# David-Wobrock/image-processing-graph-laplacian

Hardware: AMD Instinct MI355X
Metric: filtered Mpixels/sec @ 4K img, 0.5% samples; PSNR vs PETSc ref (higher is better)
Workload: dtype f32 (f32 storage and accumulation; MFMA operands split into f16 hi+lo pairs = 22 significant bits)

## Files before the change

image-processing-graph-laplacian_amd/csrc/band_plan.hpp:

```cpp
#pragma once
#include <cstdint>
#include <vector>

#if defined(__HIP__) || defined(__CUDACC__)
#define GLF_BAND_HD __host__ __device__
#else
#define GLF_BAND_HD
#endif

namespace glf {

#ifndef BAND_MAXROWS_X
#define BAND_MAXROWS_X 128
#endif
constexpr int BAND_MAXROWS = BAND_MAXROWS_X;
constexpr int BAND_RMAX = 1023;
constexpr unsigned BAND_EMPTY = 0x0000FFFFu;
#ifndef BAND_PB_X
#define BAND_PB_X 2
#endif
#ifndef BAND_NW_X
#define BAND_NW_X 8
#endif
constexpr int BAND_PB = BAND_PB_X, BAND_NW = BAND_NW_X;
constexpr int BAND_HALF_SHIFT = 3, BAND_BLOCK_SHIFT = 4, BAND_PAIR = 2;

GLF_BAND_HD inline bool band_win_live(unsigned u) { return (u & 0xFFFFu) <= (u >> 16); }
GLF_BAND_HD inline bool band_win_has(unsigned u, int c) { return c >= (int)(u & 0xFFFFu) && c <= (int)(u >> 16); }
GLF_BAND_HD inline unsigned band_win_hull(unsigned u, unsigned v)
{
    if (!band_win_live(u)) return v;
    if (!band_win_live(v)) return u;
    const unsigned lo = (u & 0xFFFFu) < (v & 0xFFFFu) ? (u & 0xFFFFu) : (v & 0xFFFFu);
    const unsigned hi = (u >> 16) > (v >> 16) ? (u >> 16) : (v >> 16);
    return lo | (hi << 16);
}
GLF_BAND_HD inline void band_rows_hull(const unsigned *rowband, int r0, int n, int *alo, int *ahi)
{
    int lo = 0xFFFF, hi = -1;
    for (int w = 0; w < n; ++w) {
        const unsigned rb = rowband[r0 + w];
        if (!band_win_live(rb)) continue;
        lo = (int)(rb & 0xFFFFu) < lo ? (int)(rb & 0xFFFFu) : lo;
        hi = (int)(rb >> 16) > hi ? (int)(rb >> 16) : hi;
    }
    *alo = lo;
    *ahi = hi;
}
GLF_BAND_HD inline void band_cols_range(const int *gcol, int nc, int cmin, int cmax, int *lo, int *count)
{
    int l = 0, h = nc;
    while (l < h) {
        const int mid = (l + h) >> 1;
        if (gcol[mid] < cmin) l = mid + 1;
        else h = mid;
    }
    const int first = l;
    h = nc;
    while (l < h) {
        const int mid = (l + h) >> 1;
        if (gcol[mid] <= cmax) l = mid + 1;
        else h = mid;
    }
    *lo = first;
    *count = l - first;
}

struct BandGeom {
    int rad = 0;
    double D2 = 0.0;
    std::vector<int> rows, cols, dcmax;
    bool init(const int *grows, int nr, const int *gcols, int nc, double s_loc);
    unsigned band_of(int r) const;
    unsigned window(int cmin, int cmax, int dr, int shift) const;
};

}
```

image-processing-graph-laplacian_amd/csrc/nystroem_band.inc:

```

#ifndef BAND_SETPRIO
#define BAND_SETPRIO 1
#endif
#ifndef BAND_PCOPY
#define BAND_PCOPY 16
#endif
#ifndef BAND_NBUF
#define BAND_NBUF 2
#endif
constexpr unsigned BAND_PSTRIDE = 4u * BAND_PCOPY;
#ifndef BAND_GROWS
#define BAND_GROWS 4
#endif
constexpr int BAND_G = BAND_GROWS;
__host__ __device__ constexpr inline int band_chunk_bytes(int mb) { return mb * 2048 + 256; }
constexpr int BAND_WB = 6;
__host__ __device__ constexpr inline int band_stage_chunks(bool samples)
{
    return samples && 2 * BAND_WB > BAND_NBUF * BAND_G ? 2 * BAND_WB : BAND_NBUF * BAND_G;
}
__host__ __device__ inline unsigned band_lds_bytes(int mb, int nw, int rad, int ksc, bool samples, bool plut = true)
{
    return (plut ? 256u * BAND_PSTRIDE : 0u) + (unsigned)band_stage_chunks(samples) * (unsigned)band_chunk_bytes(mb) + 4u * (unsigned)(rad + 1) + 64u * (unsigned)ksc + 4u * BAND_MAXROWS * (unsigned)(1 + 2 * nw) + 16u;
}
// ... 464 lines not shown
        if (qblk[BAND_NBUF - 1] <= Bhi) issued = issue(qblk[BAND_NBUF - 1], qg0[BAND_NBUF - 1], (buf + BAND_NBUF - 1) % BAND_NBUF);
        if (wvalid || noskip) {
            if (blk != cur_blk) {
                cur_blk = blk;
#pragma unroll
                for (int e = 0; e < 8; ++e) {
                    const int cb = SAMPLES ? gcs[16 * blk + 8 * half + e] : gcs[8 * blk + e];
#pragma unroll
                    for (int b = 0; b < PB; ++b) ec[b][e >> 1][e & 1] = elut[min(abs(tc[b] - cb), rad)];
                }
            }
#pragma unroll 1
            for (int slot = 0; slot < BAND_G; ++slot) {
                const int i = g0 + RP * slot;
                if (i >= nb) break;
                const unsigned u = (unsigned)__builtin_amdgcn_readfirstlane((int)wwin[wave * BAND_MAXROWS + i]);
                if (!noskip && !band_win_has(u, blk)) continue;
                ++nsteps;
                const unsigned char *sl = stage + (size_t)(buf * BAND_G + slot) * CHB;
                const int ie = SAMPLES ? i : i + half;
                const float era = ie < nb ? er_s[wave * BAND_MAXROWS + ie] : 0.f;
                kstep(sl, era, ec);
            }
        }
        if (BAND_NBUF > 2) dma_wait(issued);
        else lds_dma_drain();
        __syncthreads();
#pragma unroll
        for (int d = 0; d < BAND_NBUF - 1; ++d) {
            qblk[d] = qblk[d + 1];
            qg0[d] = qg0[d + 1];
        }
        if (qblk[BAND_NBUF - 1] <= Bhi) advance(qblk[BAND_NBUF - 1], qg0[BAND_NBUF - 1]);
        blk = qblk[0];
        g0 = qg0[0];
        buf = (buf + 1) % BAND_NBUF;
    }
    if (evaluated && lane == 0 && nsteps) atomicAdd(evaluated, nsteps * (unsigned long long)(16 * 32 * PB));

    float iv[MB], csum[MB];
#pragma unroll
    for (int j = 0; j < MB; ++j) {
        iv[j] = inv[32 * j + l31];
        csum[j] = 0.f;
    }
    if (GREY && !SAMPLES && fw) {
        if (wvalid) {
            BandFilter flt;
            flt.sig = fsig;
            flt.w = fw;
            flt.gain = fgain;
            flt.ysub = fysub;
            flt.out = fout;
            flt.zf = fzf;
            flt.corr = fcorr;
            float wv[1 + NS][MB];
#pragma unroll
            for (int k = 0; k <= NS; ++k)
#pragma unroll
                for (int j = 0; j < MB; ++j) wv[k][j] = (k == 0 ? flt.w[32 * j + l31] : flt.sig.w[(k - 1) * LD + 32 * j + l31]) * iv[j];
#pragma unroll
            for (int b = 0; b < PB; ++b) {
#pragma unroll
                for (int q = 0; q < 16; ++q) {
                    float sdot[1 + NS];
#pragma unroll
                    for (int k = 0; k <= NS; ++k) {
                        sdot[k] = 0.f;
#pragma unroll
                        for (int j = 0; j < MB; ++j) sdot[k] = fmaf(acc[b][j][q], wv[k][j], sdot[k]);
#pragma unroll
                        for (int o = 16; o > 0; o >>= 1) sdot[k] += __shfl_xor(sdot[k], o, 64);
                    }
                    const int col = (tile * PB + b) * 32 + (q & 3) + 8 * (q >> 2) + 4 * half;
                    if (l31 == 0 && col < width) {
                        const int64_t px = (int64_t)trow * width + col;
                        if (mask[px]) continue;
                        band_filter_store<1 + NS>(flt, fpix0, px, (int)tval[px], sdot);
                    }
                }
            }
        }
        return;
    }
    if (wvalid) {
#pragma unroll
        for (int b = 0; b < PB; ++b) {
#pragma unroll
            for (int q = 0; q < 16; ++q) {
                const int t = (q & 3) + 8 * (q >> 2) + 4 * half;
                if (SAMPLES) {
                    const int bi = tile * 32 + t;
                    if (bi >= nc) continue;
                    const size_t s = (size_t)trow * nc + bi;
                    const float dg = (float)degree[s];
#pragma unroll
                    for (int j = 0; j < MB; ++j)
                        out[s * out_ld + 32 * j + l31] = alpha * fmaf(dg, X[s * x_ld + 32 * j + l31], -(acc[b][j][q] * iv[j]));
                } else {
                    const int col = (tile * PB + b) * 32 + t;
                    if (col >= width) continue;
                    const int64_t px = (int64_t)trow * width + col;
                    const bool is_sample = mask[px] != 0;
                    int64_t dst;
                    if (raster) dst = px;
                    else {
                        if (is_sample) continue;
                        dst = (int64_t)p + px - (int64_t)samples_before(idx, p, (uint32_t)px);
                    }
                    const float yv = (!GREY || is_sample) ? 0.f : (float)tval[px];
#pragma unroll
                    for (int j = 0; j < MB; ++j) {
                        const float v = acc[b][j][q] * iv[j];
                        out[(size_t)dst * out_ld + 32 * j + l31] = v;
                        csum[j] = fmaf(v, yv, csum[j]);
                    }
                }
            }
        }
    }
    if (GREY && !SAMPLES && cpartial) {
        __syncthreads();
        float *red = reinterpret_cast<float *>(stage);
#pragma unroll
        for (int j = 0; j < MB; ++j) {
            const float v = csum[j] + __shfl_xor(csum[j], 32, 64);
            if (half == 0) red[wave * LD + 32 * j + l31] = v;
        }
        __syncthreads();
        if (tid < LD) {
            double tot = 0.0;
            for (int w = 0; w < NW; ++w) tot += (double)red[w * LD + tid];
            cpartial[((size_t)blockIdx.y * gridDim.x + blockIdx.x) * LD + tid] = tot;
        }
    }
}

struct BandTables {
    int rad = 0, nr = 0, nc = 0, ksc = 0, width = 0;
    int tile_px = 0, ntiles_px = 0, ntiles_s = 0;
    bool ok = false;
    DevBuf<unsigned> blob;
    size_t o_pexp = 0, o_grid = 0, o_rb_px = 0, o_win_px = 0, o_rb_s = 0, o_win_s = 0, o_dcmax = 0;
    const float *tab() const { return reinterpret_cast<const float *>(blob.p); }
    const float *pexp() const { return reinterpret_cast<const float *>(blob.p + o_pexp); }
    const int *grow() const { return reinterpret_cast<const int *>(blob.p + o_grid); }
    const int *gcol() const { return grow() + nr; }
    const unsigned *rowband_px() const { return blob.p + o_rb_px; }
    const unsigned *win_px() const { return blob.p + o_win_px; }
    const unsigned *rowband_s() const { return blob.p + o_rb_s; }
    const unsigned *win_s() const { return blob.p + o_win_s; }
    const int *dcmax() const { return reinterpret_cast<const int *>(blob.p + o_dcmax); }
    std::vector<unsigned> h_rowband_px;
    int dc0() const { return geom.dcmax.empty() ? -1 : geom.dcmax[0]; }
    int cols_near_tile(int t) const
    {
        int lo = 0, n = 0;
        if (dc0() >= 0) band_cols_range(geom.cols.data(), nc, t * tile_px - dc0(), std::min(width, (t + 1) * tile_px) - 1 + dc0(), &lo, &n);
        return n;
    }
    std::vector<double> pairs_dr;
    std::vector<double> pairs_dr_s;
    std::vector<int> hrows;
    BandGeom geom;
    unsigned band_of(int r) const { return geom.band_of(r); }
    double pairs_rows(const std::vector<double> &per_dr, int r) const
    {
        const unsigned rb = band_of(r);
        double tot = 0.0;
        for (int a = (int)(rb & 0xFFFFu); a <= (int)(rb >> 16); ++a) tot += per_dr[std::abs(r - hrows[a])];
        return tot;
    }
    mutable int memo_r0 = -1, memo_r1 = -1;
    mutable double memo_pairs = 0.0;
    double pairs_px(int row0, int row1) const
    {
        if (row0 == memo_r0 && row1 == memo_r1) return memo_pairs;
        double tot = 0.0;
        for (int r = row0; r < row1; ++r) tot += pairs_rows(pairs_dr, r);
        memo_r0 = row0;
        memo_r1 = row1;
        memo_pairs = tot;
        return tot;
    }
    double pairs_s(int a0, int a1) const
    {
        double tot = 0.0;
        for (int t = a0; t < a1; ++t) tot += pairs_rows(pairs_dr_s, hrows[t]);
        return tot;
    }
    int build(glf_ctx *ctx, const GridInfo &g, KernelCoef coef, int width_, int height, int tile_px_, bool want_px, bool want_s)
    {
        ok = false;
        if (!geom.init(g.rows.data(), g.nr, g.cols.data(), g.nc, (double)coef.s_loc)) return GLF_ERR_UNSUPPORTED;
        rad = geom.rad;
        nr = g.nr;
        nc = g.nc;
        ksc = (int)ceil_div(nc, 16);
        width = width_;
        tile_px = tile_px_;
        hrows = g.rows;
        if (nr > 65535 || ksc > 65535) return GLF_ERR_UNSUPPORTED;
        ntiles_px = want_px ? (int)ceil_div(width, tile_px) : 0;
        ntiles_s = want_s ? (int)ceil_div(nc, 32) : 0;
        const size_t n_tab = 256 + 2 * (size_t)(rad + 1);
        o_pexp = (n_tab + 3) / 4 * 4;
        o_grid = o_pexp + 256 * (size_t)BAND_PCOPY;
        o_rb_px = o_grid + (size_t)nr + nc;
        o_win_px = o_rb_px + (want_px ? (size_t)height : 0);
        o_rb_s = o_win_px + (size_t)rad * ntiles_px;
        o_win_s = o_rb_s + (want_s ? (size_t)nr : 0);
        o_dcmax = o_win_s + (size_t)rad * ntiles_s;
        std::vector<unsigned> h(o_dcmax + (size_t)rad);
        float *htab = reinterpret_cast<float *>(h.data());
        for (int e = 0; e < 256; ++e) htab[e] = (float)std::exp2(-(double)coef.s_val * e * e);
        for (int d = 0; d <= rad; ++d) {
            const double t = (double)coef.s_loc * (double)d * (double)d;
            htab[256 + d] = d < rad ? (float)std::exp2(-t) : 0.f;
            htab[256 + rad + 1 + d] = d < rad ? (float)std::exp2((double)NYS_F16_KSCALE_LOG2 - t) : 0.f;
        }
        for (int i = 0; i < 256 * BAND_PCOPY; ++i) reinterpret_cast<float *>(h.data())[o_pexp + i] = htab[i / BAND_PCOPY];
        for (int a = 0; a < nr; ++a) h[o_grid + a] = (unsigned)g.rows[a];
        for (int b = 0; b < nc; ++b) h[o_grid + nr + b] = (unsigned)g.cols[b];
        const std::vector<int> &dcmax = geom.dcmax;
        for (int dr = 0; dr < rad; ++dr) h[o_dcmax + dr] = (unsigned)dcmax[dr];
        int maxband = 0;
        if (want_px) {
            for (int r = 0; r < height; ++r) {
                const unsigned rb = band_of(r);
                h[o_rb_px + r] = rb;
                maxband = std::max(maxband, (int)(rb >> 16) - (int)(rb & 0xFFFF) + 1);
            }
            h_rowband_px.assign(h.begin() + o_rb_px, h.begin() + o_win_px);
            for (int dr = 0; dr < rad; ++dr)
                for (int t = 0; t < ntiles_px; ++t) h[o_win_px + (size_t)dr * ntiles_px + t] = geom.window(t * tile_px, std::min(width, (t + 1) * tile_px) - 1, dr, BAND_HALF_SHIFT);
            pairs_dr.assign(rad, 0.0);
            for (int dr = 0; dr < rad; ++dr) {
                if (dcmax[dr] < 0) continue;
                double n = 0.0;
                for (int b = 0; b < nc; ++b) n += (double)(std::min(width - 1, g.cols[b] + dcmax[dr]) - std::max(0, g.cols[b] - dcmax[dr]) + 1);
                pairs_dr[dr] = n;
            }
        }
        if (want_s) {
            for (int a = 0; a < nr; ++a) {
                const unsigned rb = band_of(g.rows[a]);
                h[o_rb_s + a] = rb;
                maxband = std::max(maxband, (int)(rb >> 16) - (int)(rb & 0xFFFF) + 1);
            }
            for (int dr = 0; dr < rad; ++dr)
                for (int t = 0; t < ntiles_s; ++t) h[o_win_s + (size_t)dr * ntiles_s + t] = geom.window(g.cols[t * 32], g.cols[std::min(nc, (t + 1) * 32) - 1], dr, BAND_BLOCK_SHIFT);
            pairs_dr_s.assign(rad, 0.0);
            for (int dr = 0; dr < rad; ++dr) {
                if (dcmax[dr] < 0) continue;
                double n = 0.0;
                int lo = 0, hi = 0;
                for (int b = 0; b < nc; ++b) {
                    while (lo < nc && g.cols[lo] < g.cols[b] - dcmax[dr]) ++lo;
                    while (hi < nc && g.cols[hi] <= g.cols[b] + dcmax[dr]) ++hi;
                    n += (double)(hi - lo);
                }
                pairs_dr_s[dr] = n;
            }
        }
        if (maxband + 8 > BAND_MAXROWS) return GLF_ERR_UNSUPPORTED;
        GLF_TRY(blob.alloc(ctx, h.size()));
        GLF_HIP(ctx, hipMemcpyAsync(blob.p, h.data(), sizeof(unsigned) * h.size(), hipMemcpyHostToDevice, ctx->stream));
        GLF_HIP(ctx, hipStreamSynchronize(ctx->stream));
        ok = true;
        return GLF_OK;
    }
    bool narrow(int height) const { return 2.0 * rad < 0.5 * std::min(width, height); }
};

struct BandCacheEntry {
    BandTables bt;
    std::vector<int> rows, cols;
    float s_loc = 0.f, s_val = 0.f;
    int width = 0, height = 0, tile_px = 0;
};
static void band_cache_delete(void *e) { delete reinterpret_cast<BandCacheEntry *>(e); }
static int band_tables_cached(glf_ctx *ctx, const GridInfo &g, KernelCoef coef, int width, int height, int tile_px, bool px, const BandTables **out)
{
    using Entry = BandCacheEntry;
    Entry *&e = reinterpret_cast<Entry *&>(ctx->band_cache[px ? 0 : 1]);
    if (e && e->bt.ok && e->rows == g.rows && e->cols == g.cols && e->s_loc == coef.s_loc && e->s_val == coef.s_val && e->width == width &&
        e->height == height && e->tile_px == tile_px) {
        *out = &e->bt;
        return GLF_OK;
    }
    delete e;
    e = new Entry;
    e->rows = g.rows;
    e->cols = g.cols;
    e->s_loc = coef.s_loc;
    e->s_val = coef.s_val;
    e->width = width;
    e->height = height;
    e->tile_px = tile_px;
    const int rc = e->bt.build(ctx, g, coef, width, height, tile_px, px, !px);
    if (rc != GLF_OK) {
        delete e;
        e = nullptr;
        return rc;
    }
    *out = &e->bt;
    return GLF_OK;
}

#ifndef BAND_NW_S_X
#define BAND_NW_S_X 8
#endif
constexpr int BAND_NW_S = BAND_NW_S_X;

template <int MB, int NS = 0, PixGen G = PixGen::Grey>
static int launch_band_px(glf_ctx *ctx, const BandTables &bt, const uint8_t *d_img, int row0, int nrows, const unsigned char *chunks,
                          const float *inv, float *phi, int phi_ld, const uint8_t *d_mask, const uint32_t *d_idx, unsigned p, int raster,
                          double *cpartial, unsigned long long *evaluated, const BandFilter *flt = nullptr, int64_t pix0 = 0, float nsval = 0.f)
{
    if constexpr (G != PixGen::Grey)
        if (flt || cpartial) return set_error(ctx, GLF_ERR_INVALID, "k_band: the colour and 16-bit formats have no filter epilogue");
    if constexpr (NS == 0 && G == PixGen::Grey)
        if (flt && flt->sig.nsig > 0) {
            if (flt->sig.nsig >= BANDV_MAXNC) return set_error(ctx, GLF_ERR_INVALID, "k_band: %d signal planes", flt->sig.nsig);
            return band_dispatch_planes(1 + flt->sig.nsig, [&](auto nc) -> int {
                return launch_band_px<MB, decltype(nc)::value - 1>(ctx, bt, d_img, row0, nrows, chunks, inv, phi, phi_ld, d_mask, d_idx, p, raster,
                                                                   cpartial, evaluated, flt, pix0);
            });
        }
    auto kern = k_band<MB, BAND_PB, BAND_NW, false, NS, G>;
    const unsigned lds = band_lds_bytes(MB, BAND_NW, bt.rad, bt.ksc, false, G == PixGen::Grey);
    GLF_HIP(ctx, hipFuncSetAttribute(reinterpret_cast<const void *>(kern), hipFuncAttributeMaxDynamicSharedMemorySize, (int)lds));
    const dim3 grid((unsigned)bt.ntiles_px, (unsigned)ceil_div(nrows, BAND_NW));
    hipLaunchKernelGGL(kern, grid, dim3(BAND_NW * 64), lds, ctx->stream, d_img, bt.width, row0, bt.grow(), bt.gcol(), bt.nr, bt.nc,
                       bt.ksc, bt.tab(), bt.pexp(), bt.rad, bt.rowband_px(), bt.win_px(), bt.ntiles_px, chunks, inv, phi, phi_ld, d_mask, d_idx, p, raster,
                       cpartial, (const float *)nullptr, 0, (const double *)nullptr, 0.f, evaluated, row0 + nrows, flt ? flt->w : (const float *)nullptr,
                       flt ? flt->gain : 0.f, flt ? flt->ysub : 0.f, flt ? flt->out : (uint8_t *)nullptr, flt ? flt->zf : (float *)nullptr,
                       flt ? flt->corr : (float *)nullptr, pix0, flt ? flt->sig : BandSignals{}, ctx->tune.band_noskip ? 1 : 0, nsval);
    GLF_LAUNCH_CHECK(ctx);
    return GLF_OK;
}
inline size_t band_px_wgs(const BandTables &bt, int nrows) { return (size_t)bt.ntiles_px * (size_t)ceil_div(nrows, BAND_NW); }

template <int MB, PixGen G = PixGen::Grey>
static int launch_band_samples(glf_ctx *ctx, const BandTables &bt, const uint8_t *svals, int a0, int nrows, const unsigned char *chunks,
                               const float *inv, float *Y, int y_ld, const float *X, int x_ld, const double *degree, float alpha,
                               unsigned long long *evaluated, float nsval = 0.f)
{
    auto kern = k_band<MB, 1, BAND_NW_S, true, 0, G>;
    const unsigned lds = band_lds_bytes(MB, BAND_NW_S, bt.rad, bt.ksc, true, G == PixGen::Grey);
    GLF_HIP(ctx, hipFuncSetAttribute(reinterpret_cast<const void *>(kern), hipFuncAttributeMaxDynamicSharedMemorySize, (int)lds));
    const dim3 grid((unsigned)bt.ntiles_s, (unsigned)ceil_div(nrows, BAND_NW_S));
    hipLaunchKernelGGL(kern, grid, dim3(BAND_NW_S * 64), lds, ctx->stream, svals, bt.nc, a0, bt.grow(), bt.gcol(), bt.nr, bt.nc, bt.ksc,
                       bt.tab(), bt.pexp(), bt.rad, bt.rowband_s(), bt.win_s(), bt.ntiles_s, chunks, inv, Y, y_ld, (const uint8_t *)nullptr,
                       (const uint32_t *)nullptr, 0u, 1, (double *)nullptr, X, x_ld, degree, alpha, evaluated, a0 + nrows, (const float *)nullptr, 0.f,
                       0.f, (uint8_t *)nullptr, (float *)nullptr, (float *)nullptr, (int64_t)0, BandSignals{}, 0, nsval);
    GLF_LAUNCH_CHECK(ctx);
    return GLF_OK;
}

static int band_prep(glf_ctx *ctx, const float *X, unsigned x_ld, const float *colscale, const void *svals, bool raw, int nr, int nc, int ksc, int mb,
                     unsigned char *chunks, int nch = 1)
{
    const size_t total = (size_t)nr * ksc * mb * 64;
    auto kern = raw && nch == 3 ? k_band_prep<true, 3> : raw ? k_band_prep<true> : k_band_prep<false>;
    hipLaunchKernelGGL(kern, dim3((unsigned)ceil_div((int64_t)total, 256)), dim3(256), 0, ctx->stream, X, x_ld, colscale, svals, nr, nc, ksc, mb, chunks);
    GLF_LAUNCH_CHECK(ctx);
    return GLF_OK;
}

static int band_svals(glf_ctx *ctx, const float4 *d_samples, unsigned p, DevBuf<uint8_t> &svals)
{
    GLF_TRY(svals.alloc(ctx, p));
    hipLaunchKernelGGL(k_gridop_svals, dim3((p + 255) / 256), dim3(256), 0, ctx->stream, d_samples, p, svals.p);
    GLF_LAUNCH_CHECK(ctx);
    return GLF_OK;
}
static int band_eval_zero(glf_ctx *ctx, DevBuf<unsigned long long> &dev_eval)
{
    GLF_TRY(dev_eval.alloc(ctx, 1));
    GLF_HIP(ctx, hipMemsetAsync(dev_eval.p, 0, sizeof(unsigned long long), ctx->stream));
    return GLF_OK;
}
static int band_eval_read(glf_ctx *ctx, const DevBuf<unsigned long long> &dev_eval, unsigned long long *h_eval)
{
    unsigned long long *pin_eval = ctx_pinned(ctx) ? reinterpret_cast<unsigned long long *>(ctx_pinned(ctx) + PINNED_BANDEVAL) : nullptr;
// ... 116 lines not shown
```

image-processing-graph-laplacian_amd/csrc/nystroem_band_sep.inc:

```

constexpr int BSEP_RB = 8;
constexpr int BSEP_ATILE = 128;
constexpr size_t BSEP_S_BYTES = 256u << 20;
static_assert(BSEP_RB == BAND_NW, "a block of the row pass is the rows of one workgroup of the column pass");
static_assert(BSEP_ATILE >= BAND_MAXROWS, "without BAND_NOSKIP one tile holds the band of a block of rows");

template <int NC>
__global__ __launch_bounds__(256) void k_band_sep_g(const float *__restrict__ psi, unsigned p, unsigned ld, const float *__restrict__ w,
                                                    const float *__restrict__ sig_w, const uint8_t *__restrict__ svals,
                                                    const float *__restrict__ ftab, int R, float *__restrict__ G)
{
    const unsigned s = blockIdx.x * 256 + threadIdx.x;
    if (s >= p) return;
    double acc[NC];
    band_q_row<NC>(psi + (size_t)s * ld, ld, w, sig_w, acc);
    const int v = (int)svals[s];
    for (int t = 0; t < R; t += 4) {
        const float f0 = ftab[(t + 0) * 256 + v], f1 = ftab[(t + 1) * 256 + v], f2 = ftab[(t + 2) * 256 + v], f3 = ftab[(t + 3) * 256 + v];
#pragma unroll
        for (int k = 0; k < NC; ++k) {
            const float q = (float)acc[k];
            *reinterpret_cast<float4 *>(G + ((size_t)k * p + s) * R + t) = make_float4(f0 * q, f1 * q, f2 * q, f3 * q);
        }
    }
}

__global__ __launch_bounds__(256) void k_band_sep_rows(const float *__restrict__ G, unsigned E, unsigned ncR, int nr, int row_begin, int row_end,
                                                       int srow0, const int *__restrict__ grow, const float *__restrict__ btab, int rad,
                                                       const unsigned *__restrict__ rowband, int noskip, float *__restrict__ S)
{
    __shared__ __attribute__((aligned(16))) float er_l[BSEP_ATILE][BSEP_RB];
    const int r0 = row_begin + blockIdx.y * BSEP_RB, nrb = min(BSEP_RB, row_end - r0);
    int alo, ahi;
    band_rows_hull(rowband, r0, nrb, &alo, &ahi);
    if (noskip) {
        alo = 0;
        ahi = nr - 1;
    }
    const unsigned e = blockIdx.x * 256 + threadIdx.x;
    const bool live = e < E;
    const unsigned plane = live ? e / ncR : 0u, rem = live ? e - plane * ncR : 0u;
    const float *g = G + (size_t)plane * nr * ncR + rem;
    float acc[BSEP_RB];
#pragma unroll
    for (int j = 0; j < BSEP_RB; ++j) acc[j] = 0.f;
    for (int a0 = alo; a0 <= ahi; a0 += BSEP_ATILE) {
        const int na = min(BSEP_ATILE, ahi - a0 + 1);
        __syncthreads();
        for (int i = threadIdx.x; i < na * BSEP_RB; i += 256) {
            const int dr = min(abs(r0 + i % BSEP_RB - grow[a0 + i / BSEP_RB]), rad);
            er_l[i / BSEP_RB][i % BSEP_RB] = btab[256 + rad + 1 + dr];
        }
        __syncthreads();
        if (live)
            for (int i = 0; i < na; ++i) {
                const float gv = g[(size_t)(a0 + i) * ncR];
                const float4 e0 = *reinterpret_cast<const float4 *>(&er_l[i][0]), e1 = *reinterpret_cast<const float4 *>(&er_l[i][4]);
                const float er[BSEP_RB] = {e0.x, e0.y, e0.z, e0.w, e1.x, e1.y, e1.z, e1.w};
#pragma unroll
                for (int j = 0; j < BSEP_RB; ++j) acc[j] = fmaf(er[j], gv, acc[j]);
            }
    }
    if (live)
#pragma unroll
        for (int j = 0; j < BSEP_RB; ++j)
            if (j < nrb) S[(size_t)(r0 + j - srow0) * E + e] = acc[j];
}

__host__ __device__ inline unsigned band_sep_lds_bytes(int R, int rad) { return 4u * (256u * (unsigned)(R + 1) + (unsigned)(rad + 1)); }

template <int NC, int KB>
__global__ __launch_bounds__(BAND_NW * 64) void k_band_sep_cols(const uint8_t *__restrict__ img, int width, int row_begin, int row_end, int srow0,
                                                                const int *__restrict__ gcol, int nc, const float *__restrict__ btab, int rad,
                                                                int dc0, const float *__restrict__ S, int R, const float *__restrict__ ftab,
                                                                const uint8_t *__restrict__ mask, BandFilter flt, int64_t fpix0, int noskip)
{
    constexpr int NW = BAND_NW;
    extern __shared__ __attribute__((aligned(16))) unsigned char bsdyn[];
    float *ft = reinterpret_cast<float *>(bsdyn);
    float *elut = ft + 256 * (R + 1);
    const int tid = threadIdx.x, lane = tid & 63, wave = __builtin_amdgcn_readfirstlane(tid >> 6);
    const int trow0 = row_begin + blockIdx.y * NW, ntw = min(NW, row_end - trow0);
    const int tc0 = blockIdx.x * 64, tc1 = min(width, tc0 + 64) - 1;
    for (int i = tid; i < 256 * R; i += NW * 64) ft[(i & 255) * (R + 1) + (i >> 8)] = ftab[i];
    for (int i = tid; i <= rad; i += NW * 64) elut[i] = btab[256 + i];
    int Clo = 0, W = 0;
    if (dc0 >= 0) band_cols_range(gcol, nc, tc0 - dc0, tc1 + dc0, &Clo, &W);
    __syncthreads();
    if (wave >= ntw && !noskip) return;
    const int trow = min(trow0 + wave, row_end - 1), tcol = min(tc0 + lane, width - 1);
    const int pv = (int)img[(size_t)trow * width + tcol];
    const float *fpx = ft + pv * (R + 1);
    const size_t ncR = (size_t)nc * R;
    double tot[NC];
#pragma unroll
    for (int k = 0; k < NC; ++k) {
        tot[k] = 0.0;
        const float *Srow = S + ((size_t)(trow - srow0) * NC + k) * ncR + (size_t)Clo * R;
        for (int k0 = 0; k0 < R; k0 += KB) {
            float U[KB];
#pragma unroll
            for (int t = 0; t < KB; ++t) U[t] = 0.f;
            for (int bb = 0; bb < W; ++bb) {
                const float ecv = elut[min(abs(tcol - gcol[Clo + bb]), rad)];
                const float *sp = Srow + (size_t)bb * R + k0;
#pragma unroll
                for (int t = 0; t < KB; ++t) U[t] = fmaf(ecv, sp[t], U[t]);
            }
#pragma unroll
            for (int t = 0; t < KB; ++t) tot[k] = fma((double)fpx[k0 + t], (double)U[t], tot[k]);
        }
    }

    if (wave >= ntw || tc0 + lane >= width) return;
    const int64_t px = (int64_t)trow * width + tcol;
    if (mask[px]) return;
    float sdot[NC];
#pragma unroll
    for (int k = 0; k < NC; ++k) sdot[k] = (float)(tot[k] * BAND_UNSCALE);
    band_filter_store<NC>(flt, fpix0, px, pv, sdot);
}

template <int NC, int KB>
static int band_sep_cols_launch(glf_ctx *ctx, const BandTables &bt, const uint8_t *d_img, int row0, int nrows, int srow0, const float *S, int R,
                                const float *ftab, unsigned lds, const uint8_t *d_mask, const BandFilter &flt, int64_t pix0)
{
    auto kern = k_band_sep_cols<NC, KB>;
    if (lds > 48u * 1024u) GLF_HIP(ctx, hipFuncSetAttribute(reinterpret_cast<const void *>(kern), hipFuncAttributeMaxDynamicSharedMemorySize, (int)lds));
    const dim3 grid((unsigned)bt.ntiles_px, (unsigned)ceil_div(nrows, BAND_NW));
    hipLaunchKernelGGL(kern, grid, dim3(BAND_NW * 64), lds, ctx->stream, d_img, bt.width, row0, row0 + nrows, srow0, bt.gcol(), bt.nc, bt.tab(), bt.rad,
                       bt.dc0(), S, R, ftab, d_mask, flt, pix0, ctx->tune.band_noskip ? 1 : 0);
    GLF_LAUNCH_CHECK(ctx);
    return GLF_OK;
}

static int launch_nystroem_band_sep(glf_ctx *ctx, const BandTables &bt, const uint8_t *d_img, int width, int64_t pix0, int64_t pix1,
                                    const float4 *d_samples, const uint8_t *d_mask, unsigned p, KernelCoef coef, const float *d_psi, unsigned ld,
                                    const BandFilter &flt, float *kernel_ms, uint64_t *entries_evaluated, double *mfma_flops, RowpassStats *stats)
{
    const int row0 = (int)(pix0 / width), row1 = (int)(pix1 / width), nrows = row1 - row0;
    const int ncol = 1 + flt.sig.nsig;
    if (ncol < 1 || ncol > BANDV_MAXNC || bt.width != width || p != (unsigned)bt.nr * (unsigned)bt.nc) return GLF_ERR_UNSUPPORTED;
    int R = 0;
    const float *ftab = nullptr;
    const _Float16 *Ff = nullptr;
    GLF_TRY(rank_tables(ctx, coef, &R, &ftab, &Ff));
    if (R <= 0) return GLF_ERR_UNSUPPORTED;
    const unsigned lds = band_sep_lds_bytes(R, bt.rad);
    if (lds > BANDV_LDS_MAX) return GLF_ERR_UNSUPPORTED;
    const size_t row_bytes = sizeof(float) * (size_t)bt.nc * R * ncol;
    int chunk = (int)std::min<size_t>((size_t)round_up(nrows, BAND_NW), std::max<size_t>(BAND_NW, BSEP_S_BYTES / row_bytes / BAND_NW * BAND_NW));
    DevBuf<uint8_t> svals;
    DevBuf<float> G, S;
    GLF_TRY(G.alloc(ctx, (size_t)ncol * p * R));
    while (S.alloc(ctx, (size_t)chunk * bt.nc * R * ncol) != GLF_OK) {
        if (chunk <= BAND_NW) return GLF_ERR_NOMEM;
        chunk = (int)round_up(chunk / 2, BAND_NW);
    }
    GLF_TRY(band_svals(ctx, d_samples, p, svals));
    hipStream_t st = ctx->stream;
    hipEvent_t e0 = ctx->ev[6], e1 = ctx->ev[7];
    const bool noskip = ctx->tune.band_noskip;
    GLF_TRY(band_dispatch_planes(ncol, [&](auto nc_) -> int {
        constexpr int NC = decltype(nc_)::value;
        hipLaunchKernelGGL(k_band_sep_g<NC>, dim3((p + 255) / 256), dim3(256), 0, st, d_psi, p, ld, flt.w, flt.sig.w, svals.p, ftab, R, G.p);
        GLF_LAUNCH_CHECK(ctx);
        const unsigned ncR = (unsigned)bt.nc * (unsigned)R, E = ncR * NC;
        GLF_HIP(ctx, hipEventRecord(e0, st));
        for (int c0 = 0; c0 < nrows; c0 += chunk) {
            const int r0 = row0 + c0, n = std::min(chunk, nrows - c0);
            hipLaunchKernelGGL(k_band_sep_rows, dim3((E + 255) / 256, (unsigned)ceil_div(n, BSEP_RB)), dim3(256), 0, st, G.p, E, ncR, bt.nr, r0, r0 + n, r0,
                               bt.grow(), bt.tab(), bt.rad, bt.rowband_px(), noskip ? 1 : 0, S.p);
            GLF_LAUNCH_CHECK(ctx);
            if (R % 32 == 0) GLF_TRY((band_sep_cols_launch<NC, 32>(ctx, bt, d_img, r0, n, r0, S.p, R, ftab, lds, d_mask, flt, pix0)));
            else GLF_TRY((band_sep_cols_launch<NC, 16>(ctx, bt, d_img, r0, n, r0, S.p, R, ftab, lds, d_mask, flt, pix0)));
        }
        GLF_HIP(ctx, hipEventRecord(e1, st));
        return GLF_OK;
    }));
    GLF_HIP(ctx, hipStreamSynchronize(st));
    float ms = 0.f;
    GLF_HIP(ctx, hipEventElapsedTime(&ms, e0, e1));
    if (kernel_ms) *kernel_ms = ms;
    if (entries_evaluated) {
        uint64_t cols = 0, rows = 0;
        for (int t = 0; t < bt.ntiles_px; ++t) cols += (uint64_t)bt.cols_near_tile(t);
        if (noskip) rows = (uint64_t)ceil_div(nrows, BAND_NW) * BAND_NW * (uint64_t)bt.nr;
        else
            for (int r = row0; r < row1; ++r) {
                int alo, ahi;
                band_rows_hull(bt.h_rowband_px.data(), r, 1, &alo, &ahi);
                rows += (uint64_t)std::max(0, ahi - alo + 1);
            }
        *entries_evaluated = 64ull * cols * rows;
    }
    if (mfma_flops) *mfma_flops = 0.0;
    band_stats(stats, bt, row0, row1, 1, ms, (unsigned)ncol, R);
    return GLF_OK;
}
```

Baseline: 2512.

## Move separable band column pass onto split-f16 MFMA with per-plane scaling

```diff
diff --git a/image-processing-graph-laplacian_amd/csrc/band_plan.hpp b/image-processing-graph-laplacian_amd/csrc/band_plan.hpp
--- a/image-processing-graph-laplacian_amd/csrc/band_plan.hpp
+++ b/image-processing-graph-laplacian_amd/csrc/band_plan.hpp
@@ -66,6 +66,33 @@
     *count = l - first;
 }
 
+constexpr int BSEP_KSTEP = 16;
+GLF_BAND_HD inline void band_sep_tile_cols(const int *gcol, int nc, int width, int tc0, int tile_px, int d, int *clo, int *count)
+{
+    *clo = 0;
+    *count = 0;
+    const int tc1 = (tc0 + tile_px < width ? tc0 + tile_px : width) - 1;
+    if (d >= 0 && tc1 >= tc0) band_cols_range(gcol, nc, tc0 - d, tc1 + d, clo, count);
+}
+GLF_BAND_HD inline int band_sep_ksteps(int count) { return (count + BSEP_KSTEP - 1) / BSEP_KSTEP; }
+GLF_BAND_HD inline int band_sep_col(int clo, int i, int nc) { return clo + i < nc - 1 ? clo + i : nc - 1; }
+GLF_BAND_HD inline bool band_sep_block_dead(const int *gcol, int nc, int clo, int count, int ks, int p0, int p1, int rad)
+{
+    const int i1 = BSEP_KSTEP * ks + BSEP_KSTEP - 1 < count - 1 ? BSEP_KSTEP * ks + BSEP_KSTEP - 1 : count - 1;
+    const int first = gcol[band_sep_col(clo, BSEP_KSTEP * ks, nc)], last = gcol[band_sep_col(clo, i1, nc)];
+    return first - p1 >= rad || p0 - last >= rad;
+}
+GLF_BAND_HD inline uint64_t band_sep_tile_entries(const int *gcol, int nc, int width, int tc0, int tile_px, int d, int rad, bool all)
+{
+    int clo, count;
+    band_sep_tile_cols(gcol, nc, width, tc0, tile_px, d, &clo, &count);
+    uint64_t n = 0;
+    for (int ks = 0; ks < band_sep_ksteps(count); ++ks)
+        for (int pt = 0; pt < tile_px / 32; ++pt)
+            if (all || !band_sep_block_dead(gcol, nc, clo, count, ks, tc0 + 32 * pt, tc0 + 32 * pt + 31, rad)) n += (uint64_t)BSEP_KSTEP * 32u;
+    return n;
+}
+
 struct BandGeom {
     int rad = 0;
     double D2 = 0.0;
diff --git a/image-processing-graph-laplacian_amd/csrc/nystroem_band.inc b/image-processing-graph-laplacian_amd/csrc/nystroem_band.inc
--- a/image-processing-graph-laplacian_amd/csrc/nystroem_band.inc
+++ b/image-processing-graph-laplacian_amd/csrc/nystroem_band.inc
@@ -640,6 +640,7 @@
     const unsigned *win_s() const { return blob.p + o_win_s; }
     const int *dcmax() const { return reinterpret_cast<const int *>(blob.p + o_dcmax); }
     std::vector<unsigned> h_rowband_px;
+    double er15_rowsum = 0.0;
     int dc0() const { return geom.dcmax.empty() ? -1 : geom.dcmax[0]; }
     int cols_near_tile(int t) const
     {
@@ -720,6 +721,13 @@
                 maxband = std::max(maxband, (int)(rb >> 16) - (int)(rb & 0xFFFF) + 1);
             }
             h_rowband_px.assign(h.begin() + o_rb_px, h.begin() + o_win_px);
+            er15_rowsum = 0.0;
+            for (int r = 0; r < height; ++r) {
+                const unsigned rb = h[o_rb_px + r];
+                double s = 0.0;
+                for (int a = (int)(rb & 0xFFFFu); a <= (int)(rb >> 16); ++a) s += (double)htab[256 + rad + 1 + std::min(std::abs(r - g.rows[a]), rad)];
+                er15_rowsum = std::max(er15_rowsum, s);
+            }
             for (int dr = 0; dr < rad; ++dr)
                 for (int t = 0; t < ntiles_px; ++t) h[o_win_px + (size_t)dr * ntiles_px + t] = geom.window(t * tile_px, std::min(width, (t + 1) * tile_px) - 1, dr, BAND_HALF_SHIFT);
             pairs_dr.assign(rad, 0.0);
diff --git a/image-processing-graph-laplacian_amd/csrc/nystroem_band_sep.inc b/image-processing-graph-laplacian_amd/csrc/nystroem_band_sep.inc
--- a/image-processing-graph-laplacian_amd/csrc/nystroem_band_sep.inc
+++ b/image-processing-graph-laplacian_amd/csrc/nystroem_band_sep.inc
@@ -8,12 +8,23 @@
 template <int NC>
 __global__ __launch_bounds__(256) void k_band_sep_g(const float *__restrict__ psi, unsigned p, unsigned ld, const float *__restrict__ w,
                                                     const float *__restrict__ sig_w, const uint8_t *__restrict__ svals,
-                                                    const float *__restrict__ ftab, int R, float *__restrict__ G)
-{
+                                                    const float *__restrict__ ftab, int R, float *__restrict__ G, float *__restrict__ qpart)
+{
+    __shared__ float qm[4][NC];
     const unsigned s = blockIdx.x * 256 + threadIdx.x;
-    if (s >= p) return;
+    const bool live = s < p;
     double acc[NC];
-    band_q_row<NC>(psi + (size_t)s * ld, ld, w, sig_w, acc);
+    if (live) band_q_row<NC>(psi + (size_t)s * ld, ld, w, sig_w, acc);
+#pragma unroll
+    for (int k = 0; k < NC; ++k) {
+        float m = live ? fabsf((float)acc[k]) : 0.f;
+#pragma unroll
+        for (int o = 32; o > 0; o >>= 1) m = fmaxf(m, __shfl_xor(m, o, 64));
+        if ((threadIdx.x & 63) == 0) qm[threadIdx.x >> 6][k] = m;
+    }
+    __syncthreads();
+    if (threadIdx.x < NC) qpart[(size_t)blockIdx.x * NC + threadIdx.x] = fmaxf(fmaxf(qm[0][threadIdx.x], qm[1][threadIdx.x]), fmaxf(qm[2][threadIdx.x], qm[3][threadIdx.x]));
+    if (!live) return;
     const int v = (int)svals[s];
     for (int t = 0; t < R; t += 4) {
         const float f0 = ftab[(t + 0) * 256 + v], f1 = ftab[(t + 1) * 256 + v], f2 = ftab[(t + 2) * 256 + v], f3 = ftab[(t + 3) * 256 + v];
@@ -67,69 +78,187 @@
             if (j < nrb) S[(size_t)(r0 + j - srow0) * E + e] = acc[j];
 }
 
+constexpr int BSEP_EC_LOG2 = 12;
+__global__ __launch_bounds__(256) void k_band_sep_scales(const float *__restrict__ qpart, int nblk, int ncol, float er15_rowsum, float *__restrict__ scl)
+{
+    __shared__ float sh[256];
+    for (int k = 0; k < ncol; ++k) {
+        float m = 0.f;
+        for (int i = threadIdx.x; i < nblk; i += 256) m = fmaxf(m, qpart[(size_t)i * ncol + k]);
+        __syncthreads();
+        sh[threadIdx.x] = m;
+        __syncthreads();
+        for (int o = 128; o > 0; o >>= 1) {
+            if ((int)threadIdx.x < o) sh[threadIdx.x] = fmaxf(sh[threadIdx.x], sh[threadIdx.x + o]);
+            __syncthreads();
+        }
+        if (threadIdx.x == 0) {
+            const float mx = sh[0] * er15_rowsum;
+            int e = 0;
+            if (mx > 0.f && isfinite(mx)) {
+                int ex;
+                (void)frexpf(mx, &ex);
+                e = 14 - ex;
+            }
+            e = max(-90, min(90, e));
+            scl[k] = ldexpf(1.0f, e);
+            scl[BANDV_MAXNC + k] = ldexpf(1.0f, -e - BSEP_EC_LOG2);
+        }
+    }
+}
+
+#ifndef BSEP_PT_X
+#define BSEP_PT_X 4
+#endif
+constexpr int BSEP_PT = BSEP_PT_X;
+constexpr int BSEP_KCH = 4;
+static_assert(BSEP_PT % 2 == 0 && BSEP_PT >= 2 && BSEP_PT <= 8, "a lane ends with BSEP_PT / 2 pixels");
+
 __host__ __device__ inline unsigned band_sep_lds_bytes(int R, int rad) { return 4u * (256u * (unsigned)(R + 1) + (unsigned)(rad + 1)); }
-
-template <int NC, int KB>
-__global__ __launch_bounds__(BAND_NW * 64) void k_band_sep_cols(const uint8_t *__restrict__ img, int width, int row_begin, int row_end, int srow0,
-                                                                const int *__restrict__ gcol, int nc, const float *__restrict__ btab, int rad,
-                                                                int dc0, const float *__restrict__ S, int R, const float *__restrict__ ftab,
-                                                                const uint8_t *__restrict__ mask, BandFilter flt, int64_t fpix0, int noskip)
-{
-    constexpr int NW = BAND_NW;
+__host__ __device__ inline unsigned band_sep_frag_offset(int R, int rad) { return (band_sep_lds_bytes(R, rad) + 15u) & ~15u; }
+__host__ __device__ inline unsigned band_sep_mfma_lds_bytes(int R, int rad) { return band_sep_frag_offset(R, rad) + (unsigned)(BSEP_KCH * BSEP_PT) * 2048u; }
+
+template <int NC, int PT>
+__global__ __launch_bounds__(BAND_NW * 64) void k_band_sep_cols_mfma(const uint8_t *__restrict__ img, int width, int row_begin, int row_end, int srow0,
+                                                                     const int *__restrict__ gcol, int nc, const float *__restrict__ btab, int rad,
+                                                                     int dc0, const float *__restrict__ S, int R, const float *__restrict__ ftab,
+                                                                     const float *__restrict__ scl, const uint8_t *__restrict__ mask, BandFilter flt,
+                                                                     int64_t fpix0, int noskip)
+{
+    constexpr int NW = BAND_NW, NI = PT / 2;
     extern __shared__ __attribute__((aligned(16))) unsigned char bsdyn[];
     float *ft = reinterpret_cast<float *>(bsdyn);
     float *elut = ft + 256 * (R + 1);
-    const int tid = threadIdx.x, lane = tid & 63, wave = __builtin_amdgcn_readfirstlane(tid >> 6);
+    f16x8 *bfrag = reinterpret_cast<f16x8 *>(bsdyn + band_sep_frag_offset(R, rad));
+    const int tid = threadIdx.x, lane = tid & 63, wave = __builtin_amdgcn_readfirstlane(tid >> 6), half = lane >> 5, l31 = lane & 31;
     const int trow0 = row_begin + blockIdx.y * NW, ntw = min(NW, row_end - trow0);
-    const int tc0 = blockIdx.x * 64, tc1 = min(width, tc0 + 64) - 1;
+    const int tc0 = blockIdx.x * (32 * PT);
     for (int i = tid; i < 256 * R; i += NW * 64) ft[(i & 255) * (R + 1) + (i >> 8)] = ftab[i];
     for (int i = tid; i <= rad; i += NW * 64) elut[i] = btab[256 + i];
-    int Clo = 0, W = 0;
-    if (dc0 >= 0) band_cols_range(gcol, nc, tc0 - dc0, tc1 + dc0, &Clo, &W);
+    int Clo, W;
+    band_sep_tile_cols(gcol, nc, width, tc0, 32 * PT, dc0, &Clo, &W);
+    const int nks = band_sep_ksteps(W);
+    const bool walk = wave < ntw || noskip;
+    const int trow = min(trow0 + wave, row_end - 1);
+    int pv[PT];
+#pragma unroll
+    for (int t = 0; t < PT; ++t) pv[t] = (int)img[(size_t)trow * width + min(tc0 + 32 * t + l31, width - 1)];
     __syncthreads();
-    if (wave >= ntw && !noskip) return;
-    const int trow = min(trow0 + wave, row_end - 1), tcol = min(tc0 + lane, width - 1);
-    const int pv = (int)img[(size_t)trow * width + tcol];
-    const float *fpx = ft + pv * (R + 1);
+    auto form = [&](int ks0) {
+        for (int i = tid; i < BSEP_KCH * PT * 64; i += NW * 64) {
+            const int ln = i & 63, t = (i >> 6) % PT, ks = ks0 + (i >> 6) / PT;
+            if (ks >= nks) break;
+            const int cpx = tc0 + 32 * t + (ln & 31);
+            f16x8 hi, lo;
+#pragma unroll
+            for (int j = 0; j < 8; ++j) {
+                const int e = BSEP_KSTEP * ks + 8 * (ln >> 5) + j;
+                const float ec = elut[min(abs(cpx - gcol[band_sep_col(Clo, e, nc)]), rad)];
+                const float v = e < W ? ec * (float)(1 << BSEP_EC_LOG2) : 0.f;
+                hi[j] = (_Float16)v;
+                lo[j] = (_Float16)(v - (float)hi[j]);
+            }
+            bfrag[((i >> 6) * 2 + 0) * 64 + ln] = hi;
+            bfrag[((i >> 6) * 2 + 1) * 64 + ln] = lo;
+        }
+    };
+    const bool once = nks <= BSEP_KCH;
+    if (once) {
+        form(0);
+        __syncthreads();
+    }
     const size_t ncR = (size_t)nc * R;
-    double tot[NC];
-#pragma unroll
+    float sdot[NI][NC];
+#pragma unroll 1
     for (int k = 0; k < NC; ++k) {
-        tot[k] = 0.0;
-        const float *Srow = S + ((size_t)(trow - srow0) * NC + k) * ncR + (size_t)Clo * R;
-        for (int k0 = 0; k0 < R; k0 += KB) {
-            float U[KB];
-#pragma unroll
-            for (int t = 0; t < KB; ++t) U[t] = 0.f;
-            for (int bb = 0; bb < W; ++bb) {
-                const float ecv = elut[min(abs(tcol - gcol[Clo + bb]), rad)];
-                const float *sp = Srow + (size_t)bb * R + k0;
-#pragma unroll
-                for (int t = 0; t < KB; ++t) U[t] = fmaf(ecv, sp[t], U[t]);
-            }
-#pragma unroll
-            for (int t = 0; t < KB; ++t) tot[k] = fma((double)fpx[k0 + t], (double)U[t], tot[k]);
-        }
-    }
-
-    if (wave >= ntw || tc0 + lane >= width) return;
-    const int64_t px = (int64_t)trow * width + tcol;
-    if (mask[px]) return;
-    float sdot[NC];
-#pragma unroll
-    for (int k = 0; k < NC; ++k) sdot[k] = (float)(tot[k] * BAND_UNSCALE);
-    band_filter_store<NC>(flt, fpix0, px, pv, sdot);
-}
-
-template <int NC, int KB>
+        const float sc = scl[k];
+        const float *Srow = S + ((size_t)(trow - srow0) * NC + k) * ncR;
+        double tot[PT];
+#pragma unroll
+        for (int t = 0; t < PT; ++t) tot[t] = 0.0;
+        for (int k0 = 0; k0 < R; k0 += 32) {
+            f32x16 acc[PT];
+#pragma unroll
+            for (int t = 0; t < PT; ++t)
+#pragma unroll
+                for (int q = 0; q < 16; ++q) acc[t][q] = 0.f;
+            const bool kin = k0 + l31 < R;
+            const float *Sk = Srow + min(k0 + l31, R - 1);
+            for (int ks0 = 0; ks0 < nks; ks0 += BSEP_KCH) {
+                if (!once) {
+                    __syncthreads();
+                    form(ks0);
+                    __syncthreads();
+                }
+                if (!walk) continue;
+                const int ks1 = min(ks0 + BSEP_KCH, nks);
+                float sv[8], sn[8];
+#pragma unroll
+                for (int j = 0; j < 8; ++j) sn[j] = Sk[(size_t)band_sep_col(Clo, BSEP_KSTEP * ks0 + 8 * half + j, nc) * R];
+                for (int ks = ks0; ks < ks1; ++ks) {
+#pragma unroll
+                    for (int j = 0; j < 8; ++j) sv[j] = sn[j];
+                    if (ks + 1 < ks1)
+#pragma unroll
+                        for (int j = 0; j < 8; ++j) sn[j] = Sk[(size_t)band_sep_col(Clo, BSEP_KSTEP * (ks + 1) + 8 * half + j, nc) * R];
+                    f16x8 ah, al;
+#pragma unroll
+                    for (int j = 0; j < 8; ++j) {
+                        const float v = kin ? sv[j] * sc : 0.f;
+                        ah[j] = (_Float16)v;
+                        al[j] = (_Float16)(v - (float)ah[j]);
+                    }
+                    const f16x8 *bf = bfrag + (size_t)(ks - ks0) * PT * 128 + lane;
+#pragma unroll
+                    for (int t = 0; t < PT; ++t) {
+                        if (!noskip && band_sep_block_dead(gcol, nc, Clo, W, ks, tc0 + 32 * t, tc0 + 32 * t + 31, rad)) continue;
+                        const f16x8 bh = bf[t * 128], bl = bf[t * 128 + 64];
+                        acc[t] = __builtin_amdgcn_mfma_f32_32x32x16_f16(ah, bh, acc[t], 0, 0, 0);
+                        acc[t] = __builtin_amdgcn_mfma_f32_32x32x16_f16(ah, bl, acc[t], 0, 0, 0);
+                        acc[t] = __builtin_amdgcn_mfma_f32_32x32x16_f16(al, bh, acc[t], 0, 0, 0);
+                    }
+                }
+            }
+#pragma unroll
+            for (int q = 0; q < 16; ++q) {
+                if (k0 + 8 * (q >> 2) >= R) continue;
+                const int kk = k0 + (q & 3) + 8 * (q >> 2) + 4 * half;
+#pragma unroll
+                for (int t = 0; t < PT; ++t) tot[t] = fma((double)ft[pv[t] * (R + 1) + kk], (double)acc[t][q], tot[t]);
+            }
+        }
+        const double unscale = BAND_UNSCALE * (double)scl[BANDV_MAXNC + k];
+#pragma unroll
+        for (int i = 0; i < NI; ++i) {
+            const double s0 = tot[2 * i] + __shfl_xor(tot[2 * i], 32, 64), s1 = tot[2 * i + 1] + __shfl_xor(tot[2 * i + 1], 32, 64);
+            const float r = (float)((half ? s1 : s0) * unscale);
+#pragma unroll
+            for (int kk = 0; kk < NC; ++kk)
+                if (kk == k) sdot[i][kk] = r;
+        }
+    }
+
+    if (wave >= ntw) return;
+#pragma unroll
+    for (int i = 0; i < NI; ++i) {
+        const int col = tc0 + 64 * i + lane;
+        if (col >= width) continue;
+        const int64_t px = (int64_t)trow * width + col;
+        if (mask[px]) continue;
+        band_filter_store<NC>(flt, fpix0, px, (int)img[px], sdot[i]);
+    }
+}
+
+template <int NC>
 static int band_sep_cols_launch(glf_ctx *ctx, const BandTables &bt, const uint8_t *d_img, int row0, int nrows, int srow0, const float *S, int R,
-                                const float *ftab, unsigned lds, const uint8_t *d_mask, const BandFilter &flt, int64_t pix0)
-{
-    auto kern = k_band_sep_cols<NC, KB>;
+                                const float *ftab, const float *scl, const uint8_t *d_mask, const BandFilter &flt, int64_t pix0)
+{
+    auto kern = k_band_sep_cols_mfma<NC, BSEP_PT>;
+    const unsigned lds = band_sep_mfma_lds_bytes(R, bt.rad);
     if (lds > 48u * 1024u) GLF_HIP(ctx, hipFuncSetAttribute(reinterpret_cast<const void *>(kern), hipFuncAttributeMaxDynamicSharedMemorySize, (int)lds));
-    const dim3 grid((unsigned)bt.ntiles_px, (unsigned)ceil_div(nrows, BAND_NW));
+    const dim3 grid((unsigned)ceil_div(bt.width, 32 * BSEP_PT), (unsigned)ceil_div(nrows, BAND_NW));
     hipLaunchKernelGGL(kern, grid, dim3(BAND_NW * 64), lds, ctx->stream, d_img, bt.width, row0, row0 + nrows, srow0, bt.gcol(), bt.nc, bt.tab(), bt.rad,
-                       bt.dc0(), S, R, ftab, d_mask, flt, pix0, ctx->tune.band_noskip ? 1 : 0);
+                       bt.dc0(), S, R, ftab, scl, d_mask, flt, pix0, ctx->tune.band_noskip ? 1 : 0);
     GLF_LAUNCH_CHECK(ctx);
     return GLF_OK;
 }
@@ -146,12 +275,14 @@
     const _Float16 *Ff = nullptr;
     GLF_TRY(rank_tables(ctx, coef, &R, &ftab, &Ff));
     if (R <= 0) return GLF_ERR_UNSUPPORTED;
-    const unsigned lds = band_sep_lds_bytes(R, bt.rad);
-    if (lds > BANDV_LDS_MAX) return GLF_ERR_UNSUPPORTED;
+    if (band_sep_lds_bytes(R, bt.rad) > BANDV_LDS_MAX) return GLF_ERR_UNSUPPORTED;
     const size_t row_bytes = sizeof(float) * (size_t)bt.nc * R * ncol;
     int chunk = (int)std::min<size_t>((size_t)round_up(nrows, BAND_NW), std::max<size_t>(BAND_NW, BSEP_S_BYTES / row_bytes / BAND_NW * BAND_NW));
     DevBuf<uint8_t> svals;
-    DevBuf<float> G, S;
+    DevBuf<float> G, S, qpart, scl;
+    const unsigned gblocks = (p + 255) / 256;
+    GLF_TRY(qpart.alloc(ctx, (size_t)gblocks * ncol));
+    GLF_TRY(scl.alloc(ctx, 2 * BANDV_MAXNC));
     GLF_TRY(G.alloc(ctx, (size_t)ncol * p * R));
     while (S.alloc(ctx, (size_t)chunk * bt.nc * R * ncol) != GLF_OK) {
         if (chunk <= BAND_NW) return GLF_ERR_NOMEM;
@@ -163,7 +294,9 @@
     const bool noskip = ctx->tune.band_noskip;
     GLF_TRY(band_dispatch_planes(ncol, [&](auto nc_) -> int {
         constexpr int NC = decltype(nc_)::value;
-        hipLaunchKernelGGL(k_band_sep_g<NC>, dim3((p + 255) / 256), dim3(256), 0, st, d_psi, p, ld, flt.w, flt.sig.w, svals.p, ftab, R, G.p);
+        hipLaunchKernelGGL(k_band_sep_g<NC>, dim3(gblocks), dim3(256), 0, st, d_psi, p, ld, flt.w, flt.sig.w, svals.p, ftab, R, G.p, qpart.p);
+        GLF_LAUNCH_CHECK(ctx);
+        hipLaunchKernelGGL(k_band_sep_scales, dim3(1), dim3(256), 0, st, qpart.p, (int)gblocks, NC, (float)bt.er15_rowsum, scl.p);
         GLF_LAUNCH_CHECK(ctx);
         const unsigned ncR = (unsigned)bt.nc * (unsigned)R, E = ncR * NC;
         GLF_HIP(ctx, hipEventRecord(e0, st));
@@ -172,8 +305,7 @@
             hipLaunchKernelGGL(k_band_sep_rows, dim3((E + 255) / 256, (unsigned)ceil_div(n, BSEP_RB)), dim3(256), 0, st, G.p, E, ncR, bt.nr, r0, r0 + n, r0,
                                bt.grow(), bt.tab(), bt.rad, bt.rowband_px(), noskip ? 1 : 0, S.p);
             GLF_LAUNCH_CHECK(ctx);
-            if (R % 32 == 0) GLF_TRY((band_sep_cols_launch<NC, 32>(ctx, bt, d_img, r0, n, r0, S.p, R, ftab, lds, d_mask, flt, pix0)));
-            else GLF_TRY((band_sep_cols_launch<NC, 16>(ctx, bt, d_img, r0, n, r0, S.p, R, ftab, lds, d_mask, flt, pix0)));
+            GLF_TRY(band_sep_cols_launch<NC>(ctx, bt, d_img, r0, n, r0, S.p, R, ftab, scl.p, d_mask, flt, pix0));
         }
         GLF_HIP(ctx, hipEventRecord(e1, st));
         return GLF_OK;
@@ -184,7 +316,8 @@
     if (kernel_ms) *kernel_ms = ms;
     if (entries_evaluated) {
         uint64_t cols = 0, rows = 0;
-        for (int t = 0; t < bt.ntiles_px; ++t) cols += (uint64_t)bt.cols_near_tile(t);
+        for (int tc0 = 0; tc0 < width; tc0 += 32 * BSEP_PT)
+            cols += band_sep_tile_entries(bt.geom.cols.data(), bt.nc, width, tc0, 32 * BSEP_PT, bt.dc0(), bt.rad, noskip);
         if (noskip) rows = (uint64_t)ceil_div(nrows, BAND_NW) * BAND_NW * (uint64_t)bt.nr;
         else
             for (int r = row0; r < row1; ++r) {
@@ -192,7 +325,7 @@
                 band_rows_hull(bt.h_rowband_px.data(), r, 1, &alo, &ahi);
                 rows += (uint64_t)std::max(0, ahi - alo + 1);
             }
-        *entries_evaluated = 64ull * cols * rows;
+        *entries_evaluated = cols * rows;
     }
     if (mfma_flops) *mfma_flops = 0.0;
     band_stats(stats, bt, row0, row1, 1, ms, (unsigned)ncol, R);
```

Measured after the change: 2658, median of 6. 1.06x the previous value.
